# wolearyc/ramannoodle

Hardware: NVIDIA B200
Metric: md_frames_per_s (higher is better)
Workload: dtype f64

## Files before the change

ramannoodle_b200/csrc/rn_fft.cuh:

```cuda
#pragma once

#include "rn_common.cuh"

namespace rn {
namespace fft {

constexpr int kLog2E = 12;
constexpr int kE = 1 << kLog2E;
constexpr int kNT = 256;
constexpr int kPerThread = kE / kNT;
constexpr size_t kTileSmemBytes = (size_t)kE * sizeof(double2);

enum { OUT_PLAIN = 0, OUT_POWER = 1, OUT_PEERS = 2 };

__device__ __forceinline__ double2 cmul(double2 a, double2 b) {
    return make_double2(a.x * b.x - a.y * b.y, a.x * b.y + a.y * b.x);
}
__device__ __forceinline__ double2 cadd(double2 a, double2 b) { return make_double2(a.x + b.x, a.y + b.y); }
__device__ __forceinline__ double2 csub(double2 a, double2 b) { return make_double2(a.x - b.x, a.y - b.y); }
__device__ __forceinline__ double2 conj(double2 a) { return make_double2(a.x, -a.y); }

template <int SGN>
__device__ __forceinline__ double2 mul_i(double2 a) {
    return SGN > 0 ? make_double2(-a.y, a.x) : make_double2(a.y, -a.x);
}

template <int RADIX, int SGN>
struct Dft;

template <int SGN>
struct Dft<2, SGN> {
    static __device__ __forceinline__ void run(double2* v) {
        const double2 a = v[0];
        v[0] = cadd(a, v[1]);
        v[1] = csub(a, v[1]);
    }
};

template <int SGN>
struct Dft<4, SGN> {
    static __device__ __forceinline__ void run(double2* v) {
        const double2 s02 = cadd(v[0], v[2]), d02 = csub(v[0], v[2]);
        const double2 s13 = cadd(v[1], v[3]), d13 = mul_i<SGN>(csub(v[1], v[3]));
        v[0] = cadd(s02, s13);
        v[1] = cadd(d02, d13);
        v[2] = csub(s02, s13);
        v[3] = csub(d02, d13);
    }
};

template <int SGN>
struct Dft<8, SGN> {
    static __device__ __forceinline__ void run(double2* v) {
        double2 e[4] = {v[0], v[2], v[4], v[6]};
        double2 o[4] = {v[1], v[3], v[5], v[7]};
        Dft<4, SGN>::run(e);
        Dft<4, SGN>::run(o);
        const double h = 0.70710678118654752440;
        const double2 o1 = make_double2(h * (o[1].x - SGN * o[1].y), h * (SGN * o[1].x + o[1].y));
        const double2 o2 = mul_i<SGN>(o[2]);
        const double2 o3 = make_double2(h * (-o[3].x - SGN * o[3].y), h * (SGN * o[3].x - o[3].y));
        v[0] = cadd(e[0], o[0]);
        v[4] = csub(e[0], o[0]);
        v[1] = cadd(e[1], o1);
        v[5] = csub(e[1], o1);
        v[2] = cadd(e[2], o2);
        v[6] = csub(e[2], o2);
        v[3] = cadd(e[3], o3);
        v[7] = csub(e[3], o3);
    }
};

template <int RADIX>
struct Log2;
template <>
struct Log2<2> {
    static constexpr int value = 1;
};
template <>
struct Log2<4> {
    static constexpr int value = 2;
};
template <>
struct Log2<8> {
    static constexpr int value = 3;
};

template <int RADIX>
__device__ __forceinline__ void apply_powers(double2* x, double2 w1) {
    x[1] = cmul(x[1], w1);
    if constexpr (RADIX >= 4) {
        const double2 w2 = cmul(w1, w1);
        const double2 w3 = cmul(w2, w1);
        x[2] = cmul(x[2], w2);
        x[3] = cmul(x[3], w3);
        if constexpr (RADIX == 8) {
            const double2 w4 = cmul(w2, w2);
            x[4] = cmul(x[4], w4);
            x[5] = cmul(x[5], cmul(w4, w1));
            x[6] = cmul(x[6], cmul(w3, w3));
            x[7] = cmul(x[7], cmul(w4, w3));
        }
    }
}

template <int RADIX>
__device__ __forceinline__ void apply_base_step(double2* x, double2 base, double2 step) {
    double2 w = base;
#pragma unroll
    for (int q = 0; q < RADIX; q++) {
        x[q] = cmul(x[q], w);
        if (q + 1 < RADIX) w = cmul(w, step);
    }
}

__device__ __forceinline__ int swz(int pos) { return pos ^ ((pos >> 3) & 7); }

struct Twiddles {
    const double2* hi;
    const double2* lo;
    const double2* sub;
    int split;
};

__device__ __forceinline__ double2 tw_global(const Twiddles& T, uint32_t m) {
    return cmul(__ldg(T.hi + (m >> T.split)), __ldg(T.lo + (m & ((1u << T.split) - 1u))));
}

struct PeerOut {
    double2* ptr[8];
    int log2w;
    int log2lh;
    int rank;
    int world;
    int64_t c;
};

__host__ __device__ __forceinline__ int64_t mirror_half_slots(int log2w) { return ((int64_t)1 << (log2w - 1)) + 64; }

__device__ __forceinline__ void mirror_arcs(int o, int64_t c, int log2lh, int log2w, int64_t* near_origin,
                                            int64_t* far_top) {
    const int64_t lh = (int64_t)1 << log2lh;
    const int64_t a0 = ((int64_t)o << log2w) + (c & 1);
    *near_origin = (((c + a0) >> 1) & (lh - 1)) & ~(int64_t)31;
    *far_top = (((2 * lh + c - a0) >> 1) & (lh - 1)) | 31;
}

__device__ __forceinline__ void mirror_owner(int64_t m1, int64_t c, int log2lh, int log2w, int world, int* owner,
                                             int64_t* slot) {
    const int64_t lh = (int64_t)1 << log2lh;
    int64_t u = 2 * m1 - c;
    if (u < 0) u += 2 * lh;
    const bool far_side = u > lh;
    const int64_t a = far_side ? 2 * lh - u : u;
    const int o = min((int)(a >> log2w), world - 1);
    int64_t near_origin, far_top;
    mirror_arcs(o, c, log2lh, log2w, &near_origin, &far_top);
    *owner = o;
    *slot = far_side ? mirror_half_slots(log2w) + ((far_top - m1) & (lh - 1)) : ((m1 - near_origin) & (lh - 1));
}

struct OutSpec {
    int mode;
    double* power;
    int64_t M;
    PeerOut peers;
};

__device__ __forceinline__ void store_out(const OutSpec& out, double2* plain, int seq, int64_t m, double2 v) {
    if (out.mode == OUT_PLAIN) {
        *plain = v;
    } else if (out.mode == OUT_POWER) {
        if (m < out.M) out.power[(int64_t)seq * out.M + m] = v.x * v.x + v.y * v.y;
    } else {
        int owner;
        int64_t slot;
        mirror_owner(m, out.peers.c, out.peers.log2lh, out.peers.log2w, out.peers.world, &owner, &slot);
        const int64_t stride = 2 * mirror_half_slots(out.peers.log2w);
        out.peers.ptr[owner][(int64_t)(seq * out.peers.world + out.peers.rank) * stride + slot] = v;
    }
}

template <int SGN, int RADIX, bool LEAN, class Rd, class Wr>
__device__ __forceinline__ void fft_stage(int log2sp, int log2b, const double2* __restrict__ wsub, Rd rd, Wr wr) {
    constexpr int NB = kPerThread / RADIX;
    constexpr int LR = Log2<RADIX>::value;
    const int sp = 1 << log2sp;
    const int log2ns = log2sp - log2b + LR;
    const bool has_tw = log2sp > log2b;
#pragma unroll(LEAN ? 1 : NB)
    for (int m = 0; m < NB; m++) {
        const int u = (int)threadIdx.x + m * kNT;
        const int lo = u & (sp - 1);
        const int pos0 = ((u >> log2sp) << (log2sp + LR)) + lo;
        double2 x[RADIX];
#pragma unroll
        for (int q = 0; q < RADIX; q++) x[q] = rd(pos0 + (q << log2sp), m * RADIX + q);
        double2 w1 = make_double2(1.0, 0.0);
        if (has_tw) {
            w1 = __ldg(wsub + ((lo >> log2b) << (kLog2E - log2ns)));
            if (SGN > 0) w1.y = -w1.y;
        }
        if (SGN > 0 && has_tw) apply_powers<RADIX>(x, w1);
        Dft<RADIX, SGN>::run(x);
        if (SGN < 0 && has_tw) apply_powers<RADIX>(x, w1);
#pragma unroll
        for (int q = 0; q < RADIX; q++) wr(pos0 + (q << log2sp), m * RADIX + q, x[q]);
    }
}

struct TileParams {
    double2* X;
    int64_t seq_stride;
    int tiles_per_seq;
    const double2* H;
    double2* Hout;
    int64_t limit;
    int seq_base;
    OutSpec out;
    Twiddles tw;
};

template <bool FWD_ONLY, bool LEAN>
__global__ void __launch_bounds__(kNT, LEAN ? 3 : 2) tile_kernel(const __grid_constant__ TileParams P) {
    extern __shared__ __align__(16) unsigned char fft_smem[];
    double2* S = reinterpret_cast<double2*>(fft_smem);
    const int seq = blockIdx.x / P.tiles_per_seq;
    const int tile = blockIdx.x - seq * P.tiles_per_seq;
    const int64_t tile_base = (int64_t)tile * kE;
    double2* base = P.X + (int64_t)seq * P.seq_stride + tile_base;
    const double2* wsub = P.tw.sub;

    auto rd_s = [&](int pos, int) { return S[swz(pos)]; };
    auto wr_s = [&](int pos, int, double2 v) { S[swz(pos)] = v; };
    auto rd_g = [&](int pos, int) {
        return (tile_base + pos < P.limit) ? base[pos] : make_double2(0.0, 0.0);
    };

    fft_stage<-1, 8, LEAN>(9, 0, wsub, rd_g, wr_s);
    __syncthreads();
    fft_stage<-1, 8, LEAN>(6, 0, wsub, rd_s, wr_s);
    __syncthreads();
    fft_stage<-1, 8, LEAN>(3, 0, wsub, rd_s, wr_s);
    __syncthreads();
#pragma unroll(LEAN ? 1 : kPerThread / 8)
    for (int m = 0; m < kPerThread / 8; m++) {
        const int pos0 = ((int)threadIdx.x + m * kNT) << 3;
        double2 h[8];
        const int hu = (int)threadIdx.x + m * kNT;
        if (!FWD_ONLY) {
#pragma unroll
            for (int q = 0; q < 8; q++) h[q] = __ldg(P.H + tile_base + (q << 9) + hu);
        }
        double2 x[8];
#pragma unroll
        for (int q = 0; q < 8; q++) x[q] = S[swz(pos0 + q)];
        Dft<8, -1>::run(x);
        if (FWD_ONLY) {
#pragma unroll
            for (int q = 0; q < 8; q++) P.Hout[tile_base + (q << 9) + hu] = x[q];
        } else {
#pragma unroll
            for (int q = 0; q < 8; q++) x[q] = cmul(x[q], h[q]);
            Dft<8, +1>::run(x);
#pragma unroll
            for (int q = 0; q < 8; q++) S[swz(pos0 + q)] = x[q];
        }
    }
    if (FWD_ONLY) return;
    __syncthreads();
    fft_stage<+1, 8, LEAN>(3, 0, wsub, rd_s, wr_s);
    __syncthreads();
    fft_stage<+1, 8, LEAN>(6, 0, wsub, rd_s, wr_s);
    __syncthreads();
    auto wr_g = [&](int pos, int, double2 v) { store_out(P.out, base + pos, P.seq_base + seq, tile_base + pos, v); };
    fft_stage<+1, 8, LEAN>(9, 0, wsub, rd_s, wr_g);
}

struct LevelParams {
    double2* X;
    int64_t seq_stride;
    int log2lsub;
    int log2r;
    int nsub;
    int tw_shift;
    int64_t limit;
    int seq_base;
    OutSpec out;
    Twiddles tw;
};

__device__ __forceinline__ int rev3(int x, int groups) {
    int r = 0;
    for (int i = 0; i < groups; i++) {
        r = (r << 3) | (x & 7);
        x >>= 3;
    }
    return r;
}

template <int SGN>
struct LevelCtx {
    const LevelParams& P;
    double2* S;
    double2* base;
    int64_t elem_base;
    int seq;
    int log2b, log2s;
    int a8;
    int j0;
};

template <int SGN, int RADIX, bool SMEM_SIDE, bool LEAN>
__device__ __forceinline__ void level_twiddle_stage(const LevelCtx<SGN>& C) {
    constexpr int NB = kPerThread / RADIX;
    constexpr int LR = Log2<RADIX>::value;
    const LevelParams& P = C.P;
    const int B = 1 << C.log2b;
    const int groups = (P.log2r - LR) / 3;
#pragma unroll(LEAN ? 1 : (RADIX == 8 ? NB : 2))
    for (int m = 0; m < NB; m++) {
        const int u = (int)threadIdx.x + m * kNT;
        const int col = u & (B - 1);
        const int rb = u >> C.log2b;
        const int pos0 = (rb << (C.log2b + LR)) + col;
        const uint32_t j = (uint32_t)(C.j0 + col);
        const uint32_t krest = (uint32_t)rev3(rb, groups);
        double2 wb = tw_global(P.tw, (krest * j) << P.tw_shift);
        double2 ws = tw_global(P.tw, (j << (P.log2r - LR)) << P.tw_shift);
        if (SGN > 0) {
            wb.y = -wb.y;
            ws.y = -ws.y;
        }
        double2 x[RADIX];
        if (SGN < 0) {
#pragma unroll
            for (int q = 0; q < RADIX; q++) {
                const int pos = pos0 + (q << C.log2b);
                if (SMEM_SIDE) {
                    x[q] = C.S[swz(pos)];
                } else {
                    const int64_t off = ((int64_t)(pos >> C.log2b) << C.log2s) + (pos & (B - 1));
                    x[q] = (C.elem_base + off < P.limit) ? C.base[off] : make_double2(0.0, 0.0);
                }
            }
            Dft<RADIX, SGN>::run(x);
            apply_base_step<RADIX>(x, wb, ws);
#pragma unroll
            for (int q = 0; q < RADIX; q++) {
                const int pos = pos0 + (q << C.log2b);
                C.base[((int64_t)(pos >> C.log2b) << C.log2s) + (pos & (B - 1))] = x[q];
            }
        } else {
#pragma unroll
            for (int q = 0; q < RADIX; q++) {
                const int pos = pos0 + (q << C.log2b);
                x[q] = C.base[((int64_t)(pos >> C.log2b) << C.log2s) + (pos & (B - 1))];
            }
            apply_base_step<RADIX>(x, wb, ws);
            Dft<RADIX, SGN>::run(x);
#pragma unroll
            for (int q = 0; q < RADIX; q++) {
                const int pos = pos0 + (q << C.log2b);
                if (SMEM_SIDE) {
                    C.S[swz(pos)] = x[q];
                } else {
                    const int64_t off = ((int64_t)(pos >> C.log2b) << C.log2s) + (pos & (B - 1));
                    store_out(P.out, C.base + off, C.seq, C.elem_base + off, x[q]);
                }
            }
        }
    }
}

template <int SGN, bool LEAN>
__global__ void __launch_bounds__(kNT, LEAN ? 3 : 2) level_kernel(const __grid_constant__ LevelParams P) {
    extern __shared__ __align__(16) unsigned char fft_smem[];
    double2* S = reinterpret_cast<double2*>(fft_smem);
    const int log2b = kLog2E - P.log2r;
    const int log2s = P.log2lsub - P.log2r;
    const int log2chunks = log2s - log2b;
    const int chunk = blockIdx.x & ((1 << log2chunks) - 1);
    const int rest = blockIdx.x >> log2chunks;
    const int sub = rest % P.nsub;
    const int seq = rest / P.nsub;
    const int64_t elem_base = ((int64_t)sub << P.log2lsub) + ((int64_t)chunk << log2b);
    double2* base = P.X + (int64_t)seq * P.seq_stride + elem_base;
    const double2* wsub = P.tw.sub;
    const int a8 = P.log2r / 3, r1 = P.log2r % 3;
    const int B = 1 << log2b;
    LevelCtx<SGN> C{P, S, base, elem_base, P.seq_base + seq, log2b, log2s, a8, chunk << log2b};

    auto rd_s = [&](int pos, int) { return S[swz(pos)]; };
    auto wr_s = [&](int pos, int, double2 v) { S[swz(pos)] = v; };
    auto goff = [&](int pos) { return ((int64_t)(pos >> log2b) << log2s) + (pos & (B - 1)); };

    if (a8 + (r1 ? 1 : 0) == 1) {
        if (r1 == 1) level_twiddle_stage<SGN, 2, false, LEAN>(C);
        else if (r1 == 2) level_twiddle_stage<SGN, 4, false, LEAN>(C);
        else level_twiddle_stage<SGN, 8, false, LEAN>(C);
        return;
    }
    if constexpr (SGN < 0) {
        auto rd_g = [&](int pos, int) {
            const int64_t off = goff(pos);
            return (elem_base + off < P.limit) ? base[off] : make_double2(0.0, 0.0);
        };
        int log2sp = kLog2E - 3;
        fft_stage<-1, 8, LEAN>(log2sp, log2b, wsub, rd_g, wr_s);
        __syncthreads();
        const int mid = (r1 ? a8 : a8 - 1) - 1;
        for (int i = 0; i < mid; i++) {
            log2sp -= 3;
            fft_stage<-1, 8, LEAN>(log2sp, log2b, wsub, rd_s, wr_s);
            __syncthreads();
        }
        if (r1 == 1) level_twiddle_stage<-1, 2, true, LEAN>(C);
        else if (r1 == 2) level_twiddle_stage<-1, 4, true, LEAN>(C);
        else level_twiddle_stage<-1, 8, true, LEAN>(C);
    } else {
        if (r1 == 1) level_twiddle_stage<+1, 2, true, LEAN>(C);
        else if (r1 == 2) level_twiddle_stage<+1, 4, true, LEAN>(C);
        else level_twiddle_stage<+1, 8, true, LEAN>(C);
        __syncthreads();
        const int mid = (r1 ? a8 : a8 - 1) - 1;
        int log2sp = kLog2E - 3 * (mid + 1);
        for (int i = 0; i < mid; i++) {
            fft_stage<+1, 8, LEAN>(log2sp, log2b, wsub, rd_s, wr_s);
            __syncthreads();
            log2sp += 3;
        }
        auto wr_g = [&](int pos, int, double2 v) {
            const int64_t off = goff(pos);
            store_out(P.out, base + off, P.seq_base + seq, elem_base + off, v);
        };
        fft_stage<+1, 8, LEAN>(kLog2E - 3, log2b, wsub, rd_s, wr_g);
    }
}

}
}
```

Baseline: 1.013 billion.

## Stage first-pass global loads into shared memory with cp.async in two batches

Replaces the direct global reads in the first FFT stage of the tile and level kernels, and in the inverse level twiddle stage, with cp.async copies into swizzled shared memory. The copies are committed as two groups, and the first pass waits on the first half before consuming it, so later loads stay in flight while compute starts. This aims to hide global-memory latency and cut register pressure from holding loads in flight. The cost is extra shared-memory traffic and async-copy bookkeeping, and it relies on the smem slots being written only after the matching wait.

```diff
diff --git a/ramannoodle_b200/csrc/rn_fft.cuh b/ramannoodle_b200/csrc/rn_fft.cuh
--- a/ramannoodle_b200/csrc/rn_fft.cuh
+++ b/ramannoodle_b200/csrc/rn_fft.cuh
@@ -1,6 +1,7 @@
 #pragma once
 
 #include "rn_common.cuh"
+#include "rn_device.cuh"
 
 namespace rn {
 namespace fft {
@@ -116,6 +117,30 @@
 
 __device__ __forceinline__ int swz(int pos) { return pos ^ ((pos >> 3) & 7); }
 
+template <int RADIX, class Addr, class Valid>
+__device__ __forceinline__ void land_issue(double2* S, int log2sp, Addr addr, Valid valid) {
+    constexpr int NB = kPerThread / RADIX;
+    constexpr int LR = Log2<RADIX>::value;
+#pragma unroll
+    for (int m = 0; m < NB; m++) {
+        const int u = (int)threadIdx.x + m * kNT;
+        const int pos0 = ((u >> log2sp) << (log2sp + LR)) + (u & ((1 << log2sp) - 1));
+#pragma unroll
+        for (int q = 0; q < RADIX; q++) {
+            const int pos = pos0 + (q << log2sp);
+            cp_async_16(smem_u32(S + swz(pos)), addr(pos), valid(pos) ? 16 : 0);
+        }
+        if (m == NB / 2 - 1 || m == NB - 1) cp_async_commit();
+    }
+}
+template <int RADIX>
+__device__ __forceinline__ double2 land_rd(const double2* S, int pos, int slot) {
+    constexpr int NB = kPerThread / RADIX;
+    if (slot == 0) cp_async_wait<1>();
+    else if (slot == NB / 2 * RADIX) cp_async_wait<0>();
+    return S[swz(pos)];
+}
+
 struct Twiddles {
     const double2* hi;
     const double2* lo;
@@ -233,11 +258,8 @@
 
     auto rd_s = [&](int pos, int) { return S[swz(pos)]; };
     auto wr_s = [&](int pos, int, double2 v) { S[swz(pos)] = v; };
-    auto rd_g = [&](int pos, int) {
-        return (tile_base + pos < P.limit) ? base[pos] : make_double2(0.0, 0.0);
-    };
-
-    fft_stage<-1, 8, LEAN>(9, 0, wsub, rd_g, wr_s);
+    land_issue<8>(S, 9, [&](int pos) { return base + pos; }, [&](int pos) { return tile_base + pos < P.limit; });
+    fft_stage<-1, 8, LEAN>(9, 0, wsub, [&](int pos, int slot) { return land_rd<8>(S, pos, slot); }, wr_s);
     __syncthreads();
     fft_stage<-1, 8, LEAN>(6, 0, wsub, rd_s, wr_s);
     __syncthreads();
@@ -355,7 +377,8 @@
 #pragma unroll
             for (int q = 0; q < RADIX; q++) {
                 const int pos = pos0 + (q << C.log2b);
-                x[q] = C.base[((int64_t)(pos >> C.log2b) << C.log2s) + (pos & (B - 1))];
+                x[q] = SMEM_SIDE ? land_rd<RADIX>(C.S, pos, m * RADIX + q)
+                                 : C.base[((int64_t)(pos >> C.log2b) << C.log2s) + (pos & (B - 1))];
             }
             apply_base_step<RADIX>(x, wb, ws);
             Dft<RADIX, SGN>::run(x);
@@ -402,12 +425,11 @@
         return;
     }
     if constexpr (SGN < 0) {
-        auto rd_g = [&](int pos, int) {
-            const int64_t off = goff(pos);
-            return (elem_base + off < P.limit) ? base[off] : make_double2(0.0, 0.0);
-        };
         int log2sp = kLog2E - 3;
-        fft_stage<-1, 8, LEAN>(log2sp, log2b, wsub, rd_g, wr_s);
+        land_issue<8>(S, log2sp, [&](int pos) { return base + goff(pos); },
+                      [&](int pos) { return elem_base + goff(pos) < P.limit; });
+        fft_stage<-1, 8, LEAN>(log2sp, log2b, wsub, [&](int pos, int slot) { return land_rd<8>(S, pos, slot); },
+                               wr_s);
         __syncthreads();
         const int mid = (r1 ? a8 : a8 - 1) - 1;
         for (int i = 0; i < mid; i++) {
@@ -419,6 +441,11 @@
         else if (r1 == 2) level_twiddle_stage<-1, 4, true, LEAN>(C);
         else level_twiddle_stage<-1, 8, true, LEAN>(C);
     } else {
+        auto addr = [&](int pos) { return base + goff(pos); };
+        auto all = [](int) { return true; };
+        if (r1 == 1) land_issue<2>(S, log2b, addr, all);
+        else if (r1 == 2) land_issue<4>(S, log2b, addr, all);
+        else land_issue<8>(S, log2b, addr, all);
         if (r1 == 1) level_twiddle_stage<+1, 2, true, LEAN>(C);
         else if (r1 == 2) level_twiddle_stage<+1, 4, true, LEAN>(C);
         else level_twiddle_stage<+1, 8, true, LEAN>(C);
```

New measurement: 1.006 billion, median of 6. Within noise of the previous version (-0.7%).
